# zju3dv/clean-pvnet

Hardware: NVIDIA H100
Metric: ransac_vote_throughput (higher is better)
Workload: dtype f32

## Files before the change

### clean_pvnet_b200/csrc/api.cu

```cuda
#include <cmath>
#include <cstdarg>
#include <cstdio>
#include <cstring>
#include <new>
#include <vector>
#include "kernels.h"

using namespace pvb;

namespace {

thread_local char g_err[512] = "";

int fail(int code, const char *fmt, ...)
{
    va_list ap;
    va_start(ap, fmt);
    vsnprintf(g_err, sizeof(g_err), fmt, ap);
    va_end(ap);
    return code;
}

int cuda_fail(cudaError_t e, const char *what)
{
// ... 153 lines not shown
    P->win = reinterpret_cast<float2 *>(w + L.win);
    P->refit.partial = reinterpret_cast<double *>(w + L.refit_partial);
    P->refit.ticket = reinterpret_cast<int *>(w + L.refit_ticket);
    P->refit.splits = L.refit_splits;
    P->prune.cells = reinterpret_cast<int *>(w + L.prune_cells);
    P->prune.key = reinterpret_cast<int *>(w + L.prune_key);
    P->prune.list = reinterpret_cast<int *>(w + L.prune_list);
    P->prune.len = reinterpret_cast<int *>(w + L.prune_len);
    const size_t BK = (size_t)d->B * d->K;
    const size_t prune_sub = align_up(L.prune_len + 2 * BK * sizeof(int));
    P->prune.sub = reinterpret_cast<int *>(w + prune_sub);
    P->prune.b2 = reinterpret_cast<int *>(w + align_up(prune_sub + BK * L.prune_ncells * 4 * PRUNE_REC * sizeof(int)));
    P->prune.ticket = P->refit.ticket;
    P->prune.ncx = (d->W + PRUNE_CELL - 1) / PRUNE_CELL;
    P->prune.ncells = L.prune_ncells;
    P->prune.cos_w = P->prune.sin_w = 0.f;
    return PVB_OK;
}

cudaError_t run_vote(const Plan &P, bool prune, cudaStream_t st)
{
    PruneArgs q = P.prune;
    if (prune && prune_setup(P.v, q)) return launch_vote_pruned(P.v, q, st);
    return launch_vote(P.v, false, st);
}

int run_select(const Plan &P, cudaStream_t st)
{
    cudaError_t e = cudaMemsetAsync(P.s.status, 0, P.L.bits, st);
    if (e != cudaSuccess) return cuda_fail(e, "memset(header)");
    e = launch_select(P.s, st);
    if (e != cudaSuccess) return cuda_fail(e, "select kernels");
    return PVB_OK;
}

int run_front(const Plan &P, bool prune, cudaStream_t st, ProfCall *pc)
{
    prof_start(pc, PVB_STAGE_SELECT, st);
    int rc = run_select(P, st);
    if (rc) return rc;
    prof_end(pc, PVB_STAGE_SELECT, st);
    prof_start(pc, PVB_STAGE_GENERATE, st);
    cudaError_t e = launch_generate(P.v, st);
    if (e != cudaSuccess) return cuda_fail(e, "generate kernel");
    prof_end(pc, PVB_STAGE_GENERATE, st);
    prof_start(pc, PVB_STAGE_VOTE, st);
    e = run_vote(P, prune, st);
    if (e != cudaSuccess) return cuda_fail(e, "vote kernel");
    prof_end(pc, PVB_STAGE_VOTE, st);
    return PVB_OK;
}

}

struct pvb_exchange {
    int rank, world, slots, device;
    size_t bytes_per_rank;
    size_t status_off, total;
    char *local;
    char *peer[PVB_MAX_PEERS];
    bool ipc_opened[PVB_MAX_PEERS];
    bool connected;
};

namespace {

// ... 661 lines not shown
        else if (e == cudaSuccess)
            vptr = reinterpret_cast<const float *>(vertex_alias + (size_t)b0 * vbytes);
        if (e != cudaSuccess) return cuda_fail(e, "H2D copy");
        if (stage_mask || stage_vertex) {
            e = cudaEventRecord(hp->dma[slot], hp->copy);
            if (e == cudaSuccess) e = cudaStreamWaitEvent(hp->in, hp->dma[slot], 0);
            if (e != cudaSuccess) return cuda_fail(e, "pipeline event");
        }
        pvb_desc di = dc;
        di.B = c;
        di.img_base = d->img_base + b0;
        di.capacity = Lc.capacity;
        Plan P;
        rc = make_plan(&di, mptr, vptr, nullptr, nullptr, sb + S.ws, S.end - S.ws, 1u, 2u, &P);
        if (rc) return rc;
        P.s.rowwise_gather = stage_vertex ? 0 : 1;
        rc = run_select(P, hp->in);
        if (rc) return rc;
        e = cudaEventRecord(hp->sel[slot], hp->in);
        if (e == cudaSuccess) e = cudaStreamWaitEvent(hp->cmp, hp->sel[slot], 0);
        if (e != cudaSuccess) return cuda_fail(e, "pipeline event");
        PeerPush none;
        memset(&none, 0, sizeof(none));
        e = launch_generate(P.v, hp->cmp);
        if (e == cudaSuccess) e = run_vote(P, true, hp->cmp);
        if (e == cudaSuccess) e = launch_refit(P.v, P.win, P.refit, reinterpret_cast<float *>(sb + S.out), none, hp->cmp);
        if (e != cudaSuccess) return cuda_fail(e, "compute kernels");
        e = cudaMemcpyAsync(reinterpret_cast<char *>(out_kpt_host) + (size_t)b0 * obytes, sb + S.out, (size_t)c * obytes, cudaMemcpyDeviceToHost, hp->cmp);
        if (e == cudaSuccess) e = cudaEventRecord(hp->done[slot], hp->cmp);
        if (e != cudaSuccess) return cuda_fail(e, "D2H copy");
    }
    e = cudaEventRecord(hp->end, hp->cmp);
    if (e == cudaSuccess) e = cudaStreamWaitEvent(user, hp->end, 0);
    if (e == cudaSuccess) e = cudaStreamSynchronize(user);
    if (e != cudaSuccess) return cuda_fail(e, "stream sync");
    return PVB_OK;
}

PVB_API int pvb_profile_enable(int32_t every) { g_prof_every = every < 0 ? 0 : every; g_prof_tick = 0; return PVB_OK; }

PVB_API int pvb_set_tuning(int32_t gather_mode, int32_t vote_variant)
{
    if (vote_variant < 0 || vote_variant > 3) return fail(PVB_ERR_INVALID, "vote_variant must be 0..3");
    if (gather_mode < 0 || gather_mode > 2) return fail(PVB_ERR_INVALID, "gather_mode must be 0..2");
    set_gather_tuning(gather_mode);
    set_vote_tuning(vote_variant);
    return PVB_OK;
// ... 93 lines not shown
    if (hn == 0 || vn == 0) return PVB_OK;
    if (tn == 0) {
        cudaError_t e = cudaMemsetAsync(counts, 0, sizeof(int) * (size_t)hn * vn, st);
        return e == cudaSuccess ? PVB_OK : cuda_fail(e, "memset");
    }
    if ((long long)vn * ((hn + 511) / 512) > 65535) return fail(PVB_ERR_INVALID, "vn*ceil(hn/512) must be <= 65535");
    const size_t need = pvb_vote_count_workspace_bytes(tn, vn, hn);
    if (!workspace || workspace_bytes < need) return fail(PVB_ERR_WORKSPACE, "workspace too small: need %zu", need);
    if (reinterpret_cast<uintptr_t>(workspace) & 255u) return fail(PVB_ERR_WORKSPACE, "workspace must be 256-byte aligned");
    char *w = static_cast<char *>(workspace);
    size_t off = 0;
    int *meta = reinterpret_cast<int *>(w + off); off += align_up(4 * sizeof(int));
    float2 *xy = reinterpret_cast<float2 *>(w + off); off += align_up((size_t)tn * sizeof(float2));
    float2 *dirs = reinterpret_cast<float2 *>(w + off); off += align_up((size_t)tn * vn * sizeof(float2));
    float2 *hyp_k = reinterpret_cast<float2 *>(w + off); off += align_up((size_t)hn * vn * sizeof(float2));
    int *counts_k = reinterpret_cast<int *>(w + off);
    cudaError_t e = launch_compat_repack(direct, coords, hyp, tn, vn, hn, dirs, xy, hyp_k, meta, st);
    if (e != cudaSuccess) return cuda_fail(e, "repack");
    VoteArgs v;
    memset(&v, 0, sizeof(v));
    v.B = 1; v.K = vn; v.hn = hn; v.cap = tn; v.W = 0; v.H = 0; v.thresh = inlier_thresh;
    v.tn = meta; v.state = meta + 1; v.xy = xy;
    v.dirs = dirs; v.idxs = nullptr; v.hyp = hyp_k; v.counts = counts_k;
    e = launch_vote(v, true, st);
    if (e != cudaSuccess) return cuda_fail(e, "vote kernel");
    e = launch_compat_unpack_counts(counts_k, counts, vn, hn, st);
    return e == cudaSuccess ? PVB_OK : cuda_fail(e, "unpack");
}

PVB_API int pvb_exchange_create(int32_t rank, int32_t world, int32_t slots, size_t bytes_per_rank, pvb_exchange **out)
{
    if (!out) return fail(PVB_ERR_INVALID, "out is NULL");
    *out = nullptr;
    if (world < 1 || world > PVB_MAX_PEERS || rank < 0 || rank >= world) return fail(PVB_ERR_INVALID, "bad rank %d / world %d (max %d)", rank, world, PVB_MAX_PEERS);
    if (slots < 2 || slots > 4096) return fail(PVB_ERR_INVALID, "slots must be in [2,4096]");
    if (bytes_per_rank == 0 || bytes_per_rank > ((size_t)1 << 30)) return fail(PVB_ERR_INVALID, "bad bytes_per_rank");
    pvb_exchange *ex = new (std::nothrow) pvb_exchange();
    if (!ex) return fail(PVB_ERR_INVALID, "out of host memory");
    memset(ex, 0, sizeof(*ex));
    ex->rank = rank; ex->world = world; ex->slots = slots;
    ex->bytes_per_rank = (bytes_per_rank + 15) / 16 * 16;
    ex->status_off = align_up((size_t)slots * world * ex->bytes_per_rank * 2);
    ex->total = ex->status_off + 256;
    cudaError_t e = cudaGetDevice(&ex->device);
    if (e == cudaSuccess) e = cudaMalloc(reinterpret_cast<void **>(&ex->local), ex->total);
    if (e == cudaSuccess) e = cudaMemset(ex->local, 0, ex->total);
    if (e == cudaSuccess) e = cudaDeviceSynchronize();
// ... 99 lines not shown
```

### clean_pvnet_b200/csrc/common.cuh

```cuda
#pragma once
#include <cuda_runtime.h>
#include <stdint.h>

namespace pvb {

__device__ __forceinline__ uint4 philox4x32_10(uint4 c, uint2 k)
{
#pragma unroll
    for (int r = 0; r < 10; ++r) {
        const uint32_t hi0 = __umulhi(0xD2511F53u, c.x), lo0 = 0xD2511F53u * c.x;
        const uint32_t hi1 = __umulhi(0xCD9E8D57u, c.z), lo1 = 0xCD9E8D57u * c.z;
        c = make_uint4(hi1 ^ c.y ^ k.x, lo1, hi0 ^ c.w ^ k.y, lo0);
        k.x += 0x9E3779B9u;
        k.y += 0xBB67AE85u;
    }
    return c;
}

__device__ __forceinline__ float u32_to_unit(uint32_t x) { return (float)(x >> 8) * 5.9604644775390625e-08f; }

__device__ __forceinline__ bool hypothesis_from_pair(float dx0, float dy0, float cx0, float cy0,
                                                     float dx1, float dy1, float cx1, float cy1,
                                                     float &x, float &y)
{
    const float p = __fmul_rn(dy0, dx1);
    const float q = __fmul_rn(dx0, dy1);
    const float det1 = __fsub_rn(p, q);
// ... 64 lines not shown
```

### clean_pvnet_b200/csrc/kernels.h

```cpp
#pragma once
#include <cuda_runtime.h>
#include <stdint.h>
#include "../../include/pvnet_vote_b200.h"
#include "pnp_core.cuh"

namespace pvb {

struct SelectArgs {
    const void *mask;
    int mask_dtype, select_mode;
    long long msb, msy, msx;
    const float *vertex;
    long long vs[5];
    const float *selection;
    int B, H, W, K, nwords, nblocks, cap, min_num, max_num, img_base;
    int rowwise_gather;
    int seg_classes;
    long long seg_cs;
    long long *mask_out;
    uint64_t seed;
    uint32_t tag_sel;
    uint32_t *bits;
    unsigned *blocktot;
    int *ticket;
    unsigned long long *fgsum;
    int *nz, *tn, *state, *status;
    float2 *xy, *dirs;
};
cudaError_t launch_select(const SelectArgs &a, cudaStream_t st);

struct VoteArgs {
    int B, K, hn, cap, W, H;
    float thresh;
    const int *tn;
    const int *state;
    const float2 *xy;
    const float2 *dirs;
    const int32_t *idxs;
    uint64_t seed;
    uint32_t tag_idx;
    int img_base;
    float2 *hyp;
    int *counts;
};
cudaError_t launch_generate(const VoteArgs &a, cudaStream_t st);
cudaError_t launch_vote(const VoteArgs &a, bool zero_counts, cudaStream_t st);

constexpr int PRUNE_CELL = 32;
constexpr int PRUNE_SUB = PRUNE_CELL / 2;
constexpr int PRUNE_NBIN = 128;
constexpr int PRUNE_REC = 4 + PRUNE_NBIN / 2;
constexpr int PRUNE_M = 128;
constexpr int PRUNE_MAX_HN = 2048;
constexpr int PRUNE_MIN_UNITS = 32;
static_assert(PRUNE_CELL * PRUNE_CELL < 65536, "a cell's prefix counts fit 16 bits");
struct PruneArgs {
    int *cells;
    int *sub;
    int *key;
    int *b2;
    int *list;
    int *len;
    int *ticket;
    int ncx, ncells;
    float cos_w, sin_w;
};
bool prune_setup(const VoteArgs &a, PruneArgs &q);
cudaError_t launch_vote_pruned(const VoteArgs &a, const PruneArgs &q, cudaStream_t st);
cudaError_t launch_vote_list(const VoteArgs &a, const int *list, const int *len, int max_len, cudaStream_t st);
// ... 103 lines not shown
```

### clean_pvnet_b200/csrc/prune.cu

```cuda
#include <cmath>
#include <math_constants.h>
#include "common.cuh"
#include "kernels.h"

namespace pvb {

template <bool EXACT = false>
__device__ __forceinline__ float pseudo_angle(float x, float y)
{
    const bool xn = x < 0.f, yn = y < 0.f;
    const float num = (xn == yn) ? fabsf(y) : fabsf(x), den = fabsf(x) + fabsf(y);
    const float off = yn ? (xn ? 2.f : 3.f) : (xn ? 1.f : 0.f);
    return off + (EXACT ? __fdiv_rn(num, den) : __fdividef(num, den));
}

__device__ int first_row_at(const float2 *xy, int n, float y)
{
    const int lane = threadIdx.x & 31;
    int lo = 0, hi = n;
    while (hi > lo) {
        const int step = (hi - lo + 31) / 32;
        const int p = lo + lane * step;
        const unsigned below = __ballot_sync(0xffffffffu, p < hi && __ldg(&xy[p].y) < y);
        const int nb = __popc(below);
// ... 82 lines not shown
#pragma unroll
                for (int o = 1; o < 32; o <<= 1) {
                    const int t = __shfl_up_sync(0xffffffffu, s, o);
                    if (lane >= o) s += t;
                }
                const int4 p = make_int4(s - h3 - h2 - h1, s - h3 - h2, s - h3, s);
                int *rec = q.sub + (cell * 4 + j) * PRUNE_REC;
                const bool empty = __shfl_sync(0xffffffffu, s, 31) == 0;
                if (!empty || lane == 31)
                    reinterpret_cast<int2 *>(rec + 4)[lane] = make_int2(p.x | (p.y << 16), p.z | (p.w << 16));
                if (lane < 4) {
                    const int v = s_box[sr][sx][lane];
                    if (!empty) rec[lane] = v;
                    bx = lane & 1 ? max(bx, v) : min(bx, v);
                }
                sum.x += p.x; sum.y += p.y; sum.z += p.z; sum.w += p.w;
            }
            int *rec = q.cells + cell * PRUNE_REC;
            reinterpret_cast<int2 *>(rec + 4)[lane] = make_int2(sum.x | (sum.y << 16), sum.z | (sum.w << 16));
            if (lane < 4) rec[lane] = bx;
        }
        __syncthreads();
    }
}

__device__ __forceinline__ int cell_total(const int *rec) { return (int)((unsigned)rec[PRUNE_REC - 1] >> 16); }

__device__ __forceinline__ bool bounded(float2 h) { return fabsf(h.x) + fabsf(h.y) <= 1e15f; }

__device__ __forceinline__ int bins_between(const unsigned short *P, int blo, int bhi, int tot)
{
    static_assert(PRUNE_NBIN == 128, "bins_between shifts by log2(PRUNE_NBIN)");
    auto C = [&](int j) {
        const int r = j & (PRUNE_NBIN - 1);
        return (r ? (int)P[r - 1] : 0) + tot * (j >> 7);
    };
    return C(bhi + 1) - C(blo);
}

__device__ void count_bound(const PruneArgs &q, const int *rec, int nt, float hx, float hy, int &bound)
{
    const float c = q.cos_w, s = q.sin_w;
    constexpr float EPS = 1e-5f;
    for (int t = 0; t < nt; ++t, rec += PRUNE_REC) {
        const float x0 = __int_as_float(rec[0]), x1 = __int_as_float(rec[1]);
        const float y0 = __int_as_float(rec[2]), y1 = __int_as_float(rec[3]);
// ... 160 lines not shown
            list[g + min(e, need)] = h;
            key[h] = -1;
        }
        gt += __popc(mg);
        eq += __popc(me);
    }
    if (tid == 0) q.len[bk] = M;
}

__global__ void __launch_bounds__(BOUND_THREADS, 2048 / BOUND_THREADS)
prune_bound_kernel(VoteArgs a, PruneArgs q)
{
    const int tid = threadIdx.x;
    const int part = tid / BOUND_HYPS, hl = tid % BOUND_HYPS;
    const int h = blockIdx.x * BOUND_HYPS + hl, k = blockIdx.y, b = blockIdx.z;
    const size_t bk = (size_t)b * a.K + k;
    const int tn = max(0, min(a.tn[b], a.cap));
    __shared__ __align__(16) int s_rec[2][STAGE_RECS * PRUNE_REC];
    __shared__ int s_idx[3 * BOUND_THREADS];
    __shared__ int s_part[BOUND_SPLIT][BOUND_HYPS];
    __shared__ int s_w[2 * BOUND_WARPS];
    __shared__ int s_sel[2];
    const float2 hp = (h < a.hn) ? a.hyp[bk * a.hn + h] : make_float2(0.f, 0.f);
    int bound = 0;
    stream_records<BOUND_THREADS>(q.cells + bk * q.ncells * PRUNE_REC, PRUNE_REC, q.ncells, &s_rec[0][0], s_idx, s_w,
                                  [&](const int *rec, int n) {
        const int r0 = part * n / BOUND_SPLIT, r1 = (part + 1) * n / BOUND_SPLIT;
        count_bound(q, rec + r0 * PRUNE_REC, r1 - r0, hp.x, hp.y, bound);
    });
    if (part > 0) s_part[part][hl] = bound;
    __syncthreads();
    if (part == 0 && h < a.hn) {
#pragma unroll
        for (int p = 1; p < BOUND_SPLIT; ++p) bound += s_part[p][hl];
        q.key[bk * a.hn + h] = bounded(hp) ? bound : tn;
        q.b2[bk * a.hn + h] = 0;
    }
    __threadfence();
    __syncthreads();
    if (tid == 0) {
        s_sel[0] = (atomicAdd(q.ticket + bk, 1) == (int)gridDim.x - 1);
        if (s_sel[0]) q.ticket[bk] = 0;
    }
    __syncthreads();
    if (!s_sel[0]) return;
    __threadfence();
// ... 21 lines not shown
    *total = tot;
    return before + __popc(m & ((1u << lane) - 1u));
}

__global__ void __launch_bounds__(NEXT_THREADS)
prune_next_kernel(VoteArgs a, PruneArgs q)
{
    const int x = blockIdx.x, k = blockIdx.y, b = blockIdx.z, tid = threadIdx.x;
    const size_t bk = (size_t)b * a.K + k;
    const size_t BK = (size_t)a.B * a.K;
    const int hn = a.hn;
    __shared__ __align__(16) int s_rec[2 * STAGE_RECS * PRUNE_REC];
    __shared__ int s_idx[3 * NEXT_THREADS];
    __shared__ int s_warp[NEXT_THREADS / 32];
    __shared__ int s_last;
    extern __shared__ __align__(16) unsigned char s_dyn[];
    const int ncap = hn - PRUNE_M;
    float2 *s_hyp = reinterpret_cast<float2 *>(s_dyn);
    int *s_b2 = reinterpret_cast<int *>(s_hyp + ncap);
    unsigned short *s_cand = reinterpret_cast<unsigned short *>(s_b2 + ncap);
    const int *key = q.key + bk * hn;
    const float2 *hyp = a.hyp + bk * hn;
    int *b2 = q.b2 + bk * hn;
    int L = 0;
    {
        const int *counts = a.counts + bk * hn;
        int best = 0;
        const int n1 = q.len[bk];
        for (int s = tid; s < n1; s += NEXT_THREADS) best = max(best, counts[q.list[bk * hn + s]]);
        best = __reduce_max_sync(0xffffffffu, best);
        if ((tid & 31) == 0) s_warp[tid >> 5] = best;
        __syncthreads();
        for (int w = 0; w < NEXT_THREADS / 32; ++w) L = max(L, s_warp[w]);
    }
    int nc = 0;
    for (int h0 = 0; h0 < hn && L > 0; h0 += NEXT_THREADS) {
        const int h = h0 + tid;
        const float2 hp = h < hn ? hyp[h] : make_float2(0.f, 0.f);
        const bool f = h < hn && key[h] >= L && bounded(hp);
        int n;
        const int pos = nc + cta_scan(f, s_warp, &n);
        if (f) { s_cand[pos] = (unsigned short)h; s_hyp[pos] = hp; s_b2[pos] = 0; }
        nc += n;
    }
    if (nc > 0) {
        __syncthreads();
        const int P = max(1, NEXT_THREADS / nc);
        const int *sub = q.sub + (bk * q.ncells * 4 + x) * PRUNE_REC;
        const int nsub = (4 * q.ncells - x + NEXT_CTAS - 1) / NEXT_CTAS;
        stream_records<NEXT_THREADS>(sub, NEXT_CTAS * PRUNE_REC, nsub, s_rec, s_idx, s_warp, [&](const int *rec, int n) {
            for (int it = tid; it < nc * P; it += NEXT_THREADS) {
                const int j = it % nc, p = it / nc;
// ... 28 lines not shown
        base += n;
    }
    if (tid == 0) q.len[BK + bk] = base;
}

bool prune_setup(const VoteArgs &a, PruneArgs &q)
{
    const double t = (double)a.thresh;
    if (!(t > 0.0 && t < 1.0) || a.hn <= PRUNE_M || a.hn > PRUNE_MAX_HN) return false;
    if ((long long)a.B * a.K < PRUNE_MIN_UNITS) return false;
    if ((long long)a.K * ((a.hn + 63) / 64) > 65535) return false;
    const double u = ldexp(1.0, -24);
    const double w = acos(fmax(-1.0, t - 64.0 * u)) + 1e-5;
    if (!(w < 1.5)) return false;
    q.cos_w = nextafterf((float)cos(w), 0.f);
    q.sin_w = nextafterf((float)sin(w), 1.f);
    return true;
}

cudaError_t launch_vote_pruned(const VoteArgs &a, const PruneArgs &q, cudaStream_t st)
{
    const size_t BK = (size_t)a.B * a.K;
    const int nbands = (a.H + PRUNE_CELL - 1) / PRUNE_CELL;
    prune_hist_kernel<<<dim3(nbands, a.K, a.B), HIST_THREADS, 0, st>>>(a, q);
    prune_bound_kernel<<<dim3((a.hn + BOUND_HYPS - 1) / BOUND_HYPS, a.K, a.B), BOUND_THREADS, 0, st>>>(a, q);
    cudaError_t e = launch_vote_list_slices(a, q.list, q.len, PRUNE_M, st);
    if (e != cudaSuccess) return e;
    prune_next_kernel<<<dim3(NEXT_CTAS, a.K, a.B), NEXT_THREADS, (a.hn - PRUNE_M) * NEXT_CAND_BYTES, st>>>(a, q);
    return launch_vote_list(a, q.list + BK * a.hn, q.len + BK, a.hn - PRUNE_M, st);
}

}
```

### clean_pvnet_b200/csrc/vote.cu

```cuda
#include <atomic>
#include <math_constants.h>
#include "common.cuh"
#include "kernels.h"

namespace pvb {

__global__ void __launch_bounds__(256)
generate_kernel(VoteArgs a)
{
    const int h = blockIdx.x * 256 + threadIdx.x;
    if (h >= a.hn) return;
    const int k = blockIdx.y, b = blockIdx.z;
    const int tn = min(a.tn[b], a.cap);
    float x = 0.f, y = 0.f;
    if (tn > 0) {
        int t0, t1;
        if (a.idxs) {
            const int2 t = __ldg(reinterpret_cast<const int2 *>(a.idxs) + ((size_t)b * a.hn + h) * a.K + k);
            t0 = t.x; t1 = t.y;
        } else {
            const uint4 r = philox4x32_10(make_uint4((uint32_t)h, (uint32_t)k, (uint32_t)(a.img_base + b), a.tag_idx),
                                          make_uint2((uint32_t)a.seed, (uint32_t)(a.seed >> 32)));
            t0 = (int)(r.x % (uint32_t)tn);
            t1 = (int)(r.y % (uint32_t)tn);
        }
        if ((unsigned)t0 < (unsigned)tn && (unsigned)t1 < (unsigned)tn) {
            const float2 *dk = a.dirs + ((size_t)b * a.K + k) * a.cap;
            const float2 *xy = a.xy + (size_t)b * a.cap;
            const float2 d0 = dk[t0], d1 = dk[t1], c0 = xy[t0], c1 = xy[t1];
            float hx, hy;
            if (hypothesis_from_pair(d0.x, d0.y, c0.x, c0.y, d1.x, d1.y, c1.x, c1.y, hx, hy)) { x = hx; y = hy; }
        }
    }
    a.hyp[((size_t)b * a.K + k) * a.hn + h] = make_float2(x, y);
    a.counts[((size_t)b * a.K + k) * a.hn + h] = 0;
}

cudaError_t launch_generate(const VoteArgs &a, cudaStream_t st)
{
    dim3 g((a.hn + 255) / 256, a.K, a.B);
    generate_kernel<<<g, 256, 0, st>>>(a);
    return cudaGetLastError();
}

struct VoteK {
    VoteArgs a;
    ConeParams cone;
    const int *list;
    const int *len;
};

constexpr int VOTE_BLOCK = 16;

__device__ __forceinline__ float4 lds128(uint32_t addr)
{
    float4 v;
    asm volatile("ld.shared.v4.f32 {%0,%1,%2,%3}, [%4];" : "=f"(v.x), "=f"(v.y), "=f"(v.z), "=f"(v.w) : "r"(addr) : "memory");
    return v;
}

__device__ __forceinline__ float cone_margin(const float4 ra, const float2 rb, float hxc, float hyc)
{
    const float ap = fmaf(ra.x, hxc, fmaf(ra.y, hyc, ra.z));
    const float pp = fmaf(ra.w, hxc, fmaf(rb.x, hyc, rb.y));
    return ap - fabsf(pp);
// ... 56 lines not shown
    const float S = fabsf(xc) + fabsf(yc) + cmax;
    float d = fmaxf(cone.band * S, cone.floor);
    if (!(S <= 1e15f) || !(d < CUDART_INF_F)) { xc = 0.f; yc = 0.f; d = CUDART_INF_F; }
    return make_float3(xc, yc, d);
}

template <int HPT, int NT, int MINB, int VOTE_TILE, int WS>
__global__ void __launch_bounds__(NT, MINB)
vote_kernel(const VoteK p)
{
    constexpr int PPT = VOTE_TILE / NT;
    constexpr int NW = NT / 32;
    constexpr int TEAM = WS * 32;
    constexpr int TEAMS = NT / TEAM;
    __shared__ __align__(16) float4 s_a[VOTE_TILE];
    __shared__ __align__(16) float2 s_b[VOTE_TILE];
    __shared__ float s_box[4][NW];
    const VoteArgs &a = p.a;
    const int b = blockIdx.z;
    const int k = blockIdx.y % a.K, slice = blockIdx.y / a.K;
    const int tn = min(a.tn[b], a.cap);
    const int t0 = blockIdx.x * VOTE_TILE;
    const size_t bk = (size_t)b * a.K + k;
    const int nh = p.list ? __ldg(p.len + bk) : a.hn;
    if (t0 >= tn || slice * (TEAM * HPT) >= nh) return;
    const int *lst = p.list ? p.list + bk * a.hn : nullptr;
    const int n = min(VOTE_TILE, tn - t0);
    const int npad = (n + VOTE_BLOCK - 1) / VOTE_BLOCK * VOTE_BLOCK;
    const int tid = threadIdx.x, lane = tid & 31;
    const float kappa = p.cone.kappa, thresh = p.cone.thresh;
    const float2 *hyp = a.hyp + bk * a.hn;
    const float2 *xy = a.xy + (size_t)b * a.cap + t0;
    const float2 *dk = a.dirs + ((size_t)b * a.K + k) * a.cap + t0;
    const int team = tid / TEAM;
    const int hbase = slice * (TEAM * HPT) + (tid - team * TEAM);

    float2 v[PPT], c[PPT];
    float ox, oy, cmax;
    load_tile<NT, PPT>(dk, xy, n, v, c, s_box, ox, oy, cmax);

#pragma unroll
    for (int r = 0; r < PPT; ++r) {
        const int i = tid + r * NT;
        if (i < npad) {
            float4 ra;
            float2 rb;
            cone_record(i < n, v[r], c[r], ox, oy, cmax, kappa, ra, rb);
            s_a[i] = ra; s_b[i] = rb;
        }
    }

    float hxc[HPT], hyc[HPT], dl[HPT];
    int neg[HPT];
#pragma unroll
    for (int j = 0; j < HPT; ++j) {
        const int s = hbase + j * TEAM;
        const float2 q = (s < nh) ? hyp[lst ? __ldg(lst + s) : s] : make_float2(0.f, 0.f);
        const float3 f = hyp_frame(q, ox, oy, cmax, p.cone);
        hxc[j] = f.x; hyc[j] = f.y; dl[j] = f.z;
        neg[j] = 0;
    }
    __syncthreads();

    const uint32_t sa0 = (uint32_t)__cvta_generic_to_shared(s_a);
    const uint32_t sb0 = (uint32_t)__cvta_generic_to_shared(s_b);
    int mine = 0;
    for (int i0 = team * VOTE_BLOCK; i0 < npad; i0 += TEAMS * VOTE_BLOCK) {
        mine += VOTE_BLOCK;
        const uint32_t sa = sa0 + (uint32_t)i0 * 16u, sb = sb0 + (uint32_t)i0 * 8u;
        float mn[HPT];
#pragma unroll
        for (int j = 0; j < HPT; ++j) mn[j] = CUDART_INF_F;
#pragma unroll
        for (int u = 0; u < VOTE_BLOCK; u += 2) {
            const float4 ra0 = lds128(sa + u * 16), ra1 = lds128(sa + u * 16 + 16);
            const float4 rbb = lds128(sb + u * 8);
#pragma unroll
            for (int j = 0; j < HPT; ++j) {
                const float m0 = cone_margin(ra0, make_float2(rbb.x, rbb.y), hxc[j], hyc[j]);
                const float m1 = cone_margin(ra1, make_float2(rbb.z, rbb.w), hxc[j], hyc[j]);
// ... 2 lines not shown
                mn[j] = fminf(mn[j], fminf(fabsf(m0), fabsf(m1)));
            }
        }
        bool flag = false;
#pragma unroll
        for (int j = 0; j < HPT; ++j) flag |= mn[j] < dl[j];
        if (__any_sync(0xffffffffu, flag)) {
            const int nb = min(VOTE_BLOCK, n - i0);
            float4 ra = make_float4(0.f, 0.f, -1e30f, 0.f);
            float2 rb = make_float2(0.f, 0.f), vv = make_float2(0.f, 0.f), cc = make_float2(0.f, 0.f);
            if (lane < nb) {
                ra = s_a[i0 + lane]; rb = s_b[i0 + lane];
                vv = __ldg(dk + i0 + lane); cc = __ldg(xy + i0 + lane);
            }
#pragma unroll
            for (int j = 0; j < HPT; ++j) {
                unsigned bm = __ballot_sync(0xffffffffu, mn[j] < dl[j]);
                while (bm) {
                    const int L = __ffs(bm) - 1;
                    bm &= bm - 1;
                    const float hx_ = __shfl_sync(0xffffffffu, hxc[j], L), hy_ = __shfl_sync(0xffffffffu, hyc[j], L);
                    const float dl_ = __shfl_sync(0xffffffffu, dl[j], L);
                    const int s = hbase - lane + L + j * TEAM;
                    const float2 q = (s < nh) ? __ldg(hyp + (lst ? __ldg(lst + s) : s)) : make_float2(0.f, 0.f);
                    int delta = 0;
                    if (lane < nb) {
                        const float m = cone_margin(ra, rb, hx_, hy_);
                        if (fabsf(m) < dl_) {
                            const bool in = vote_exact(vv.x, vv.y, cc.x, cc.y, q.x, q.y, thresh);
                            delta = (in ? 0 : 1) - (int)(__float_as_uint(m) >> 31);
                        }
                    }
                    delta = __reduce_add_sync(0xffffffffu, delta);
                    if (lane == L) neg[j] += delta;
                }
            }
        }
    }
    int *counts = a.counts + bk * a.hn;
#pragma unroll
    for (int j = 0; j < HPT; ++j) {
        const int s = hbase + j * TEAM;
        const int cnt = mine - neg[j];
        if (s < nh && cnt) atomicAdd(counts + (lst ? __ldg(lst + s) : s), cnt);
    }
}

ConeParams make_cone(float thresh)
{
    ConeParams c;
    c.thresh = thresh;
    const double t = (double)thresh;
    if (t > 0.0 && t < 1.0) {
        const double s = sqrt(1.0 - t * t);
        const double kappa = s / t, G = 1.0 / (t * s);
        const double band = 1.25 * ldexp(1.0, -24) * (18.0 + 22.0 * kappa + 9.0 * G);
        c.kappa = (float)kappa;
        c.band = nextafterf((float)band, INFINITY);
        c.floor = nextafterf((float)(2e-6 * (kappa + 1.0)), INFINITY);
    } else {
        c.kappa = 0.f;
        c.band = INFINITY;
        c.floor = INFINITY;
    }
    return c;
}

static std::atomic<int> g_vote_variant{0};

void set_vote_tuning(int variant) { g_vote_variant.store(variant, std::memory_order_relaxed); }

cudaError_t launch_vote(const VoteArgs &a, bool zero_counts, cudaStream_t st)
{
    if (zero_counts) {
        cudaError_t e = cudaMemsetAsync(a.counts, 0, sizeof(int) * (size_t)a.B * a.K * a.hn, st);
        if (e != cudaSuccess) return e;
    }
    VoteK p;
    p.a = a;
    p.cone = make_cone(a.thresh);
    p.list = nullptr;
    p.len = nullptr;
    const int variant = g_vote_variant.load(std::memory_order_relaxed);
#define PVB_VOTE(HPT, NT, MINB, TILE, WS)                                               \
    do {                                                                                \
        const int slices = (a.hn + (HPT) * (WS) * 32 - 1) / ((HPT) * (WS) * 32);        \
        dim3 g((a.cap + (TILE) - 1) / (TILE), a.K * slices, a.B);                       \
        vote_kernel<HPT, NT, MINB, TILE, WS><<<g, NT, 0, st>>>(p);                      \
    } while (0)
    if (a.hn <= 32) PVB_VOTE(1, 128, 8, 512, 1);
    else if (a.hn <= 64) PVB_VOTE(2, 128, 8, 512, 1);
    else if (a.hn <= 128) PVB_VOTE(4, 128, 8, 512, 1);
    else if (a.hn <= 256) PVB_VOTE(4, 128, 8, 512, 2);
    else if (variant == 2) PVB_VOTE(4, 128, 8, 256, 4);
    else if (variant == 3) PVB_VOTE(4, 128, 8, 512, 4);
    else PVB_VOTE(4, 128, 8, 1024, 4);
#undef PVB_VOTE
    return cudaGetLastError();
}

constexpr int LIST_NT = 128;
constexpr int LIST_PPT = 8;
constexpr int LIST_TILE = LIST_NT * LIST_PPT;
constexpr int LIST_CHUNK = LIST_NT;
constexpr int LIST_U = 2;
static_assert(LIST_CHUNK % LIST_U == 0 && LIST_U % 2 == 0, "");

__device__ __forceinline__ int list_exact(const float4 q, const float4 *s_a, const float2 *s_b, const float2 *hyp, const float2 *dk,
                                          const float2 *xy, int n, float thresh)
{
    const float2 hq = __ldg(hyp + __float_as_int(q.w));
    int d = 0;
    for (int i = threadIdx.x; i < n; i += LIST_NT) {
        const float m = cone_margin(s_a[i], s_b[i], q.x, q.y);
        if (fabsf(m) < q.z) {
            const float2 vv = __ldg(dk + i), cc = __ldg(xy + i);
            d += (vote_exact(vv.x, vv.y, cc.x, cc.y, hq.x, hq.y, thresh) ? 0 : 1) - (int)(__float_as_uint(m) >> 31);
        }
    }
    return d;
}

__global__ void __launch_bounds__(LIST_NT, 5)
vote_list_kernel(const VoteArgs a, const ConeParams cone, const int *__restrict__ list, const int *__restrict__ len)
{
    constexpr int NW = LIST_NT / 32;
    __shared__ __align__(16) float4 s_a[LIST_TILE];
    __shared__ __align__(16) float2 s_b[LIST_TILE];
    __shared__ __align__(16) float4 s_h[LIST_CHUNK];
    __shared__ unsigned s_tally[NW][LIST_CHUNK / 2];
    __shared__ float s_box[4][NW];
    const int b = blockIdx.z;
    const int k = blockIdx.y;
    const int tn = min(a.tn[b], a.cap);
    const int t0 = blockIdx.x * LIST_TILE;
    const size_t bk = (size_t)b * a.K + k;
    const int nh = __ldg(len + bk);
    if (t0 >= tn || nh <= 0) return;
    const int n = min(LIST_TILE, tn - t0);
    const int tid = threadIdx.x, lane = tid & 31, warp = tid >> 5;
    const int *lst = list + bk * a.hn;
    const float2 *hyp = a.hyp + bk * a.hn;
    const float2 *xy = a.xy + (size_t)b * a.cap + t0;
    const float2 *dk = a.dirs + bk * a.cap + t0;

    int h = 0;
    float2 hq = make_float2(0.f, 0.f);
    if (tid < nh) { h = __ldg(lst + tid); hq = hyp[h]; }
    float4 ra[LIST_PPT];
    float2 rb[LIST_PPT];
    float ox, oy, cmax;
    {
        float2 v[LIST_PPT], c[LIST_PPT];
        load_tile<LIST_NT, LIST_PPT>(dk, xy, n, v, c, s_box, ox, oy, cmax);
#pragma unroll
        for (int r = 0; r < LIST_PPT; ++r) {
            cone_record(tid + r * LIST_NT < n, v[r], c[r], ox, oy, cmax, cone.kappa, ra[r], rb[r]);
            s_a[tid + r * LIST_NT] = ra[r]; s_b[tid + r * LIST_NT] = rb[r];
        }
    }
    unsigned *tally = s_tally[warp];
    for (int c0 = 0; c0 < nh; c0 += LIST_CHUNK) {
        const int ns = min(LIST_CHUNK, nh - c0);
        if (c0 > 0 && tid < ns) { h = __ldg(lst + c0 + tid); hq = hyp[h]; }
        if (tid < ns) {
            const float3 f = hyp_frame(hq, ox, oy, cmax, cone);
            s_h[tid] = make_float4(f.x, f.y, f.z, __int_as_float(h));
        } else {
            s_h[tid] = make_float4(0.f, 0.f, 0.f, 0.f);
        }
        __syncthreads();
        for (int s = 0; s < ns; s += LIST_U) {
            float4 q[LIST_U];
            int neg[LIST_U];
            float mn[LIST_U];
            bool flag = false;
#pragma unroll
            for (int u = 0; u < LIST_U; ++u) {
                q[u] = s_h[s + u];
                neg[u] = 0;
                mn[u] = CUDART_INF_F;
#pragma unroll
                for (int r = 0; r < LIST_PPT; ++r) {
                    const float m = cone_margin(ra[r], rb[r], q[u].x, q[u].y);
                    neg[u] += (int)(__float_as_uint(m) >> 31);
                    mn[u] = fminf(mn[u], fabsf(m));
                }
// ... 4 lines not shown
                for (int u = 0; u < LIST_U; ++u)
                    if (mn[u] < q[u].z) neg[u] += list_exact(q[u], s_a, s_b, hyp, dk, xy, n, cone.thresh);
            }
#pragma unroll
            for (int u = 0; u < LIST_U; u += 2) {
                const unsigned t = __reduce_add_sync(0xffffffffu, (unsigned)(LIST_PPT - neg[u]) | ((unsigned)(LIST_PPT - neg[u + 1]) << 16));
                if (lane == 0) tally[(s + u) / 2] = t;
            }
        }
        __syncthreads();
        if (tid < ns) {
            int cnt = 0;
#pragma unroll
            for (int w = 0; w < NW; ++w) cnt += (int)((s_tally[w][tid / 2] >> (16 * (tid & 1))) & 0xffffu);
            if (cnt) atomicAdd(a.counts + bk * a.hn + __float_as_int(s_h[tid].w), cnt);
        }
    }
}

cudaError_t launch_vote_list(const VoteArgs &a, const int *list, const int *len, int max_len, cudaStream_t st)
{
    if (max_len <= 0) return cudaSuccess;
    dim3 g((a.cap + LIST_TILE - 1) / LIST_TILE, a.K, a.B);
    vote_list_kernel<<<g, LIST_NT, 0, st>>>(a, make_cone(a.thresh), list, len);
    return cudaGetLastError();
}

cudaError_t launch_vote_list_slices(const VoteArgs &a, const int *list, const int *len, int max_len, cudaStream_t st)
{
    constexpr int HPT = 4, NT = 128, TILE = 1024;
    static_assert(HPT * 32 == PRUNE_M, "pass 1 is one slice");
    if (max_len <= 0) return cudaSuccess;
    VoteK p;
    p.a = a;
    p.cone = make_cone(a.thresh);
    p.list = list;
    p.len = len;
    const int slices = (max_len + HPT * 32 - 1) / (HPT * 32);
    dim3 g((a.cap + TILE - 1) / TILE, a.K * slices, a.B);
    vote_kernel<HPT, NT, 8, TILE, 1><<<g, NT, 0, st>>>(p);
    return cudaGetLastError();
}

template <int NV>
__device__ __forceinline__ void peer_push(const PeerPush &pp, size_t bk, const float (&v)[NV])
{
    for (int r = 0; r < pp.world; ++r) {
        uint2 *dst = pp.recv[r] + bk * NV;
#pragma unroll
        for (int i = 0; i < NV; ++i)
            asm volatile("st.volatile.global.v2.u32 [%0], {%1, %2};" ::"l"(dst + i), "r"(__float_as_uint(v[i])), "r"(pp.seq) : "memory");
    }
}

constexpr int RF_THREADS = 128;
constexpr int RF_CHUNK = 2048;

int refit_splits_for(int cap) { return (cap + RF_CHUNK - 1) / RF_CHUNK; }

__device__ __forceinline__ bool vote_winner(float vx, float vy, float cx, float cy, float hx, float hy,
                                            const ConeParams &cone)
{
    const float dx = __fsub_rn(hx, cx), dy = __fsub_rn(hy, cy);
    const float n1sq = fmaf(vx, vx, vy * vy);
    const float S = fabsf(dx) + fabsf(dy);
    const float m = cone.kappa * fmaf(vx, dx, vy * dy) - fabsf(fmaf(vx, dy, -(vy * dx)));
    const float thr = cone.band * S;
    const bool safe = (n1sq > 1e-10f) && (n1sq < 1e8f) && (S >= 2e-6f) && (S <= 1e6f) &&
                      (m * m > thr * thr * n1sq * 1.0001f);
    return safe ? (m > 0.f) : vote_exact(vx, vy, cx, cy, hx, hy, cone.thresh);
}

__global__ void __launch_bounds__(RF_THREADS)
refit_kernel(VoteArgs a, float2 *__restrict__ win, RefitScratch rs, float *__restrict__ out, ConeParams cone, PeerPush pp)
{
    const int split = blockIdx.x, k = blockIdx.y, b = blockIdx.z;
    const int tid = threadIdx.x, lane = tid & 31, warp = tid >> 5;
    constexpr int NW = RF_THREADS / 32;
    const int tn = min(a.tn[b], a.cap);
    const size_t bk = (size_t)b * a.K + k;
    __shared__ int s_c[NW], s_h[NW];
    __shared__ double s_acc[NW][5];
    __shared__ int s_last;
    float2 res = make_float2(0.f, 0.f);
    if (a.state[b] != 0 || tn <= 0) {
        if (split != 0) return;
        if (tid == 0) { out[bk * 2] = 0.f; out[bk * 2 + 1] = 0.f; win[bk] = make_float2(0.f, 0.f); }
    } else {
        const int nsplit = (tn + RF_CHUNK - 1) / RF_CHUNK;
        if (split >= nsplit) return;
        const int *counts = a.counts + bk * a.hn;
        int bc = -1, bh = 0x7fffffff;
        for (int h = tid; h < a.hn; h += RF_THREADS) {
            const int c = counts[h];
            if (c > bc) { bc = c; bh = h; }
        }
#pragma unroll
        for (int o = 16; o > 0; o >>= 1) {
// ... 48 lines not shown
        if (!s_last) return;
        if (tid == 0) {
            __threadfence();
            double s[5] = {0, 0, 0, 0, 0};
            for (int sp = 0; sp < nsplit; ++sp)
                for (int i = 0; i < 5; ++i) s[i] += __ldcg(rs.partial + (bk * rs.splits + sp) * 5 + i);
            const double det = s[0] * s[2] - s[1] * s[1];
            float x, y;
            if (det == 0.0 || !isfinite(det)) { x = (float)s[3]; y = (float)s[4]; }
            else { x = (float)((s[2] * s[3] - s[1] * s[4]) / det); y = (float)((s[0] * s[4] - s[1] * s[3]) / det); }
            out[bk * 2] = x; out[bk * 2 + 1] = y;
            res = make_float2(x, y);
        }
    }
    if (pp.world <= 0 || tid != 0) return;
    const float v[2] = {res.x, res.y};
    peer_push<2>(pp, bk, v);
}

cudaError_t launch_refit(const VoteArgs &a, float2 *win, const RefitScratch &rs, float *out_kpt, const PeerPush &pp,
                         cudaStream_t st)
{
    dim3 g(rs.splits, a.K, a.B);
    refit_kernel<<<g, RF_THREADS, 0, st>>>(a, win, rs, out_kpt, make_cone(a.thresh), pp);
    return cudaGetLastError();
}

constexpr int CV_THREADS = 256;

__global__ void __launch_bounds__(CV_THREADS)
covariance_kernel(VoteArgs a, const float *__restrict__ mean, float *__restrict__ cov, PeerPush pp)
{
    const int k = blockIdx.x, b = blockIdx.y;
    const int tid = threadIdx.x, lane = tid & 31, warp = tid >> 5;
    const size_t bk = (size_t)b * a.K + k;
    const int tn = min(a.tn[b], a.cap);
    const bool skipped = a.state[b] != 0;
    const int *counts = a.counts + bk * a.hn;
    const float2 *hyp = a.hyp + bk * a.hn;
    const float ftn = (float)tn;
    __shared__ float s_max[CV_THREADS / 32];
    __shared__ double s_acc[CV_THREADS / 32][4];
    float mx = -CUDART_INF_F;
    bool has_nan = false;
    for (int h = tid; h < a.hn; h += CV_THREADS) {
        const float r = skipped ? 1.f : __fdiv_rn((float)counts[h], ftn);
        if (r != r) has_nan = true;
        mx = fmaxf(mx, r);
// ... 42 lines not shown
```

Measured before the change: 291,100.

## Chain select-generate-vote-refit kernels with programmatic dependent launch

Launches the generate, prune, vote and refit kernels through cudaLaunchKernelEx with programmatic stream serialization and adds griddepcontrol wait/launch_dependents calls, so each kernel's prologue (index math, point loads) overlaps the tail of the previous one. This targets launch gaps and tail bubbles in a chain of small kernels. Loads of data produced by earlier kernels are moved after the wait and switched from __ldg to __ldcg so they do not read stale non-coherent cache lines. The risk is ordering bugs if any dependent read lands before the wait.

```diff
diff --git a/clean_pvnet_b200/csrc/api.cu b/clean_pvnet_b200/csrc/api.cu
--- a/clean_pvnet_b200/csrc/api.cu
+++ b/clean_pvnet_b200/csrc/api.cu
@@ -199,7 +199,7 @@
 {
     PruneArgs q = P.prune;
     if (prune && prune_setup(P.v, q)) return launch_vote_pruned(P.v, q, st);
-    return launch_vote(P.v, false, st);
+    return launch_vote(P.v, false, false, st);
 }
 
 int run_select(const Plan &P, cudaStream_t st)
@@ -218,7 +218,7 @@
     if (rc) return rc;
     prof_end(pc, PVB_STAGE_SELECT, st);
     prof_start(pc, PVB_STAGE_GENERATE, st);
-    cudaError_t e = launch_generate(P.v, st);
+    cudaError_t e = launch_generate(P.v, true, st);
     if (e != cudaSuccess) return cuda_fail(e, "generate kernel");
     prof_end(pc, PVB_STAGE_GENERATE, st);
     prof_start(pc, PVB_STAGE_VOTE, st);
@@ -926,7 +926,7 @@
         if (e != cudaSuccess) return cuda_fail(e, "pipeline event");
         PeerPush none;
         memset(&none, 0, sizeof(none));
-        e = launch_generate(P.v, hp->cmp);
+        e = launch_generate(P.v, false, hp->cmp);
         if (e == cudaSuccess) e = run_vote(P, true, hp->cmp);
         if (e == cudaSuccess) e = launch_refit(P.v, P.win, P.refit, reinterpret_cast<float *>(sb + S.out), none, hp->cmp);
         if (e != cudaSuccess) return cuda_fail(e, "compute kernels");
@@ -1066,7 +1066,7 @@
     v.B = 1; v.K = vn; v.hn = hn; v.cap = tn; v.W = 0; v.H = 0; v.thresh = inlier_thresh;
     v.tn = meta; v.state = meta + 1; v.xy = xy;
     v.dirs = dirs; v.idxs = nullptr; v.hyp = hyp_k; v.counts = counts_k;
-    e = launch_vote(v, true, st);
+    e = launch_vote(v, true, false, st);
     if (e != cudaSuccess) return cuda_fail(e, "vote kernel");
     e = launch_compat_unpack_counts(counts_k, counts, vn, hn, st);
     return e == cudaSuccess ? PVB_OK : cuda_fail(e, "unpack");
diff --git a/clean_pvnet_b200/csrc/common.cuh b/clean_pvnet_b200/csrc/common.cuh
--- a/clean_pvnet_b200/csrc/common.cuh
+++ b/clean_pvnet_b200/csrc/common.cuh
@@ -1,8 +1,29 @@
 #pragma once
 #include <cuda_runtime.h>
 #include <stdint.h>
+#include <utility>
 
 namespace pvb {
+
+__device__ __forceinline__ void grid_dep_wait() { asm volatile("griddepcontrol.wait;" ::: "memory"); }
+__device__ __forceinline__ void grid_dep_launch_dependents() { asm volatile("griddepcontrol.launch_dependents;" ::: "memory"); }
+
+template <typename... Params, typename... Args>
+cudaError_t launch_chained(bool chained, void (*kernel)(Params...), dim3 grid, dim3 block, size_t smem, cudaStream_t st,
+                           Args &&...args)
+{
+    cudaLaunchConfig_t cfg = {};
+    cfg.gridDim = grid;
+    cfg.blockDim = block;
+    cfg.dynamicSmemBytes = smem;
+    cfg.stream = st;
+    cudaLaunchAttribute attr[1];
+    attr[0].id = cudaLaunchAttributeProgrammaticStreamSerialization;
+    attr[0].val.programmaticStreamSerializationAllowed = chained ? 1 : 0;
+    cfg.attrs = attr;
+    cfg.numAttrs = 1;
+    return cudaLaunchKernelEx(&cfg, kernel, std::forward<Args>(args)...);
+}
 
 __device__ __forceinline__ uint4 philox4x32_10(uint4 c, uint2 k)
 {
diff --git a/clean_pvnet_b200/csrc/kernels.h b/clean_pvnet_b200/csrc/kernels.h
--- a/clean_pvnet_b200/csrc/kernels.h
+++ b/clean_pvnet_b200/csrc/kernels.h
@@ -43,8 +43,8 @@
     float2 *hyp;
     int *counts;
 };
-cudaError_t launch_generate(const VoteArgs &a, cudaStream_t st);
-cudaError_t launch_vote(const VoteArgs &a, bool zero_counts, cudaStream_t st);
+cudaError_t launch_generate(const VoteArgs &a, bool chained, cudaStream_t st);
+cudaError_t launch_vote(const VoteArgs &a, bool zero_counts, bool chained, cudaStream_t st);
 
 constexpr int PRUNE_CELL = 32;
 constexpr int PRUNE_SUB = PRUNE_CELL / 2;
diff --git a/clean_pvnet_b200/csrc/prune.cu b/clean_pvnet_b200/csrc/prune.cu
--- a/clean_pvnet_b200/csrc/prune.cu
+++ b/clean_pvnet_b200/csrc/prune.cu
@@ -128,6 +128,8 @@
         }
         __syncthreads();
     }
+    grid_dep_wait();
+    grid_dep_launch_dependents();
 }
 
 __device__ __forceinline__ int cell_total(const int *rec) { return (int)((unsigned)rec[PRUNE_REC - 1] >> 16); }
@@ -334,6 +336,8 @@
     __shared__ int s_w[2 * BOUND_WARPS];
     __shared__ int s_sel[2];
     const float2 hp = (h < a.hn) ? a.hyp[bk * a.hn + h] : make_float2(0.f, 0.f);
+    grid_dep_wait();
+    grid_dep_launch_dependents();
     int bound = 0;
     stream_records<BOUND_THREADS>(q.cells + bk * q.ncells * PRUNE_REC, PRUNE_REC, q.ncells, &s_rec[0][0], s_idx, s_w,
                                   [&](const int *rec, int n) {
@@ -401,12 +405,16 @@
     const int *key = q.key + bk * hn;
     const float2 *hyp = a.hyp + bk * hn;
     int *b2 = q.b2 + bk * hn;
+    static_assert(PRUNE_M <= NEXT_THREADS, "one pass-1 entry per thread");
     int L = 0;
     {
         const int *counts = a.counts + bk * hn;
         int best = 0;
         const int n1 = q.len[bk];
-        for (int s = tid; s < n1; s += NEXT_THREADS) best = max(best, counts[q.list[bk * hn + s]]);
+        const int h1 = tid < n1 ? q.list[bk * hn + tid] : -1;
+        grid_dep_wait();
+        grid_dep_launch_dependents();
+        if (h1 >= 0) best = __ldcg(counts + h1);
         best = __reduce_max_sync(0xffffffffu, best);
         if ((tid & 31) == 0) s_warp[tid >> 5] = best;
         __syncthreads();
@@ -481,11 +489,15 @@
 {
     const size_t BK = (size_t)a.B * a.K;
     const int nbands = (a.H + PRUNE_CELL - 1) / PRUNE_CELL;
-    prune_hist_kernel<<<dim3(nbands, a.K, a.B), HIST_THREADS, 0, st>>>(a, q);
-    prune_bound_kernel<<<dim3((a.hn + BOUND_HYPS - 1) / BOUND_HYPS, a.K, a.B), BOUND_THREADS, 0, st>>>(a, q);
-    cudaError_t e = launch_vote_list_slices(a, q.list, q.len, PRUNE_M, st);
+    cudaError_t e = launch_chained(true, prune_hist_kernel, dim3(nbands, a.K, a.B), HIST_THREADS, 0, st, a, q);
+    if (e == cudaSuccess)
+        e = launch_chained(true, prune_bound_kernel, dim3((a.hn + BOUND_HYPS - 1) / BOUND_HYPS, a.K, a.B), BOUND_THREADS, 0, st,
+                           a, q);
+    if (e == cudaSuccess) e = launch_vote_list_slices(a, q.list, q.len, PRUNE_M, st);
+    if (e == cudaSuccess)
+        e = launch_chained(true, prune_next_kernel, dim3(NEXT_CTAS, a.K, a.B), NEXT_THREADS,
+                           (size_t)(a.hn - PRUNE_M) * NEXT_CAND_BYTES, st, a, q);
     if (e != cudaSuccess) return e;
-    prune_next_kernel<<<dim3(NEXT_CTAS, a.K, a.B), NEXT_THREADS, (a.hn - PRUNE_M) * NEXT_CAND_BYTES, st>>>(a, q);
     return launch_vote_list(a, q.list + BK * a.hn, q.len + BK, a.hn - PRUNE_M, st);
 }
 
diff --git a/clean_pvnet_b200/csrc/vote.cu b/clean_pvnet_b200/csrc/vote.cu
--- a/clean_pvnet_b200/csrc/vote.cu
+++ b/clean_pvnet_b200/csrc/vote.cu
@@ -8,6 +8,8 @@
 __global__ void __launch_bounds__(256)
 generate_kernel(VoteArgs a)
 {
+    grid_dep_wait();
+    grid_dep_launch_dependents();
     const int h = blockIdx.x * 256 + threadIdx.x;
     if (h >= a.hn) return;
     const int k = blockIdx.y, b = blockIdx.z;
@@ -36,11 +38,10 @@
     a.counts[((size_t)b * a.K + k) * a.hn + h] = 0;
 }
 
-cudaError_t launch_generate(const VoteArgs &a, cudaStream_t st)
+cudaError_t launch_generate(const VoteArgs &a, bool chained, cudaStream_t st)
 {
     dim3 g((a.hn + 255) / 256, a.K, a.B);
-    generate_kernel<<<g, 256, 0, st>>>(a);
-    return cudaGetLastError();
+    return launch_chained(chained, generate_kernel, g, 256, 0, st, a);
 }
 
 struct VoteK {
@@ -143,8 +144,7 @@
     const int tn = min(a.tn[b], a.cap);
     const int t0 = blockIdx.x * VOTE_TILE;
     const size_t bk = (size_t)b * a.K + k;
-    const int nh = p.list ? __ldg(p.len + bk) : a.hn;
-    if (t0 >= tn || slice * (TEAM * HPT) >= nh) return;
+    if (t0 >= tn) { grid_dep_wait(); return; }
     const int *lst = p.list ? p.list + bk * a.hn : nullptr;
     const int n = min(VOTE_TILE, tn - t0);
     const int npad = (n + VOTE_BLOCK - 1) / VOTE_BLOCK * VOTE_BLOCK;
@@ -171,12 +171,17 @@
         }
     }
 
+    grid_dep_wait();
+    grid_dep_launch_dependents();
+    const int nh = p.list ? __ldcg(p.len + bk) : a.hn;
+    if (slice * (TEAM * HPT) >= nh) return;
+
     float hxc[HPT], hyc[HPT], dl[HPT];
     int neg[HPT];
 #pragma unroll
     for (int j = 0; j < HPT; ++j) {
         const int s = hbase + j * TEAM;
-        const float2 q = (s < nh) ? hyp[lst ? __ldg(lst + s) : s] : make_float2(0.f, 0.f);
+        const float2 q = (s < nh) ? hyp[lst ? __ldcg(lst + s) : s] : make_float2(0.f, 0.f);
         const float3 f = hyp_frame(q, ox, oy, cmax, p.cone);
         hxc[j] = f.x; hyc[j] = f.y; dl[j] = f.z;
         neg[j] = 0;
@@ -225,7 +230,7 @@
                     const float hx_ = __shfl_sync(0xffffffffu, hxc[j], L), hy_ = __shfl_sync(0xffffffffu, hyc[j], L);
                     const float dl_ = __shfl_sync(0xffffffffu, dl[j], L);
                     const int s = hbase - lane + L + j * TEAM;
-                    const float2 q = (s < nh) ? __ldg(hyp + (lst ? __ldg(lst + s) : s)) : make_float2(0.f, 0.f);
+                    const float2 q = (s < nh) ? __ldg(hyp + (lst ? __ldcg(lst + s) : s)) : make_float2(0.f, 0.f);
                     int delta = 0;
                     if (lane < nb) {
                         const float m = cone_margin(ra, rb, hx_, hy_);
@@ -245,7 +250,7 @@
     for (int j = 0; j < HPT; ++j) {
         const int s = hbase + j * TEAM;
         const int cnt = mine - neg[j];
-        if (s < nh && cnt) atomicAdd(counts + (lst ? __ldg(lst + s) : s), cnt);
+        if (s < nh && cnt) atomicAdd(counts + (lst ? __ldcg(lst + s) : s), cnt);
     }
 }
 
@@ -273,7 +278,7 @@
 
 void set_vote_tuning(int variant) { g_vote_variant.store(variant, std::memory_order_relaxed); }
 
-cudaError_t launch_vote(const VoteArgs &a, bool zero_counts, cudaStream_t st)
+cudaError_t launch_vote(const VoteArgs &a, bool zero_counts, bool chained, cudaStream_t st)
 {
     if (zero_counts) {
         cudaError_t e = cudaMemsetAsync(a.counts, 0, sizeof(int) * (size_t)a.B * a.K * a.hn, st);
@@ -285,11 +290,12 @@
     p.list = nullptr;
     p.len = nullptr;
     const int variant = g_vote_variant.load(std::memory_order_relaxed);
+    cudaError_t e = cudaSuccess;
 #define PVB_VOTE(HPT, NT, MINB, TILE, WS)                                               \
     do {                                                                                \
         const int slices = (a.hn + (HPT) * (WS) * 32 - 1) / ((HPT) * (WS) * 32);        \
         dim3 g((a.cap + (TILE) - 1) / (TILE), a.K * slices, a.B);                       \
-        vote_kernel<HPT, NT, MINB, TILE, WS><<<g, NT, 0, st>>>(p);                      \
+        e = launch_chained(chained, vote_kernel<HPT, NT, MINB, TILE, WS>, g, NT, 0, st, p); \
     } while (0)
     if (a.hn <= 32) PVB_VOTE(1, 128, 8, 512, 1);
     else if (a.hn <= 64) PVB_VOTE(2, 128, 8, 512, 1);
@@ -299,7 +305,7 @@
     else if (variant == 3) PVB_VOTE(4, 128, 8, 512, 4);
     else PVB_VOTE(4, 128, 8, 1024, 4);
 #undef PVB_VOTE
-    return cudaGetLastError();
+    return e;
 }
 
 constexpr int LIST_NT = 128;
@@ -335,10 +341,12 @@
     __shared__ float s_box[4][NW];
     const int b = blockIdx.z;
     const int k = blockIdx.y;
+    grid_dep_wait();
+    grid_dep_launch_dependents();
     const int tn = min(a.tn[b], a.cap);
     const int t0 = blockIdx.x * LIST_TILE;
     const size_t bk = (size_t)b * a.K + k;
-    const int nh = __ldg(len + bk);
+    const int nh = __ldcg(len + bk);
     if (t0 >= tn || nh <= 0) return;
     const int n = min(LIST_TILE, tn - t0);
     const int tid = threadIdx.x, lane = tid & 31, warp = tid >> 5;
@@ -349,7 +357,7 @@
 
     int h = 0;
     float2 hq = make_float2(0.f, 0.f);
-    if (tid < nh) { h = __ldg(lst + tid); hq = hyp[h]; }
+    if (tid < nh) { h = __ldcg(lst + tid); hq = hyp[h]; }
     float4 ra[LIST_PPT];
     float2 rb[LIST_PPT];
     float ox, oy, cmax;
@@ -365,7 +373,7 @@
     unsigned *tally = s_tally[warp];
     for (int c0 = 0; c0 < nh; c0 += LIST_CHUNK) {
         const int ns = min(LIST_CHUNK, nh - c0);
-        if (c0 > 0 && tid < ns) { h = __ldg(lst + c0 + tid); hq = hyp[h]; }
+        if (c0 > 0 && tid < ns) { h = __ldcg(lst + c0 + tid); hq = hyp[h]; }
         if (tid < ns) {
             const float3 f = hyp_frame(hq, ox, oy, cmax, cone);
             s_h[tid] = make_float4(f.x, f.y, f.z, __int_as_float(h));
@@ -416,8 +424,7 @@
 {
     if (max_len <= 0) return cudaSuccess;
     dim3 g((a.cap + LIST_TILE - 1) / LIST_TILE, a.K, a.B);
-    vote_list_kernel<<<g, LIST_NT, 0, st>>>(a, make_cone(a.thresh), list, len);
-    return cudaGetLastError();
+    return launch_chained(true, vote_list_kernel, g, LIST_NT, 0, st, a, make_cone(a.thresh), list, len);
 }
 
 cudaError_t launch_vote_list_slices(const VoteArgs &a, const int *list, const int *len, int max_len, cudaStream_t st)
@@ -432,8 +439,7 @@
     p.len = len;
     const int slices = (max_len + HPT * 32 - 1) / (HPT * 32);
     dim3 g((a.cap + TILE - 1) / TILE, a.K * slices, a.B);
-    vote_kernel<HPT, NT, 8, TILE, 1><<<g, NT, 0, st>>>(p);
-    return cudaGetLastError();
+    return launch_chained(true, vote_kernel<HPT, NT, 8, TILE, 1>, g, NT, 0, st, p);
 }
 
 template <int NV>
@@ -468,6 +474,7 @@
 __global__ void __launch_bounds__(RF_THREADS)
 refit_kernel(VoteArgs a, float2 *__restrict__ win, RefitScratch rs, float *__restrict__ out, ConeParams cone, PeerPush pp)
 {
+    grid_dep_wait();
     const int split = blockIdx.x, k = blockIdx.y, b = blockIdx.z;
     const int tid = threadIdx.x, lane = tid & 31, warp = tid >> 5;
     constexpr int NW = RF_THREADS / 32;
@@ -562,8 +569,7 @@
                          cudaStream_t st)
 {
     dim3 g(rs.splits, a.K, a.B);
-    refit_kernel<<<g, RF_THREADS, 0, st>>>(a, win, rs, out_kpt, make_cone(a.thresh), pp);
-    return cudaGetLastError();
+    return launch_chained(true, refit_kernel, g, RF_THREADS, 0, st, a, win, rs, out_kpt, make_cone(a.thresh), pp);
 }
 
 constexpr int CV_THREADS = 256;
```

Result: faster. 300,600, median of 6 (+3.3%).
